# atunnd/Hair-centric-Image-Retrieval

Hardware: AMD Instinct MI355X
Metric: query-images/sec (embed+top-10) ViT-B/16 vs 1M gallery, 1/2/4/8 GPU (higher is better)
Workload: dtype f16; 1 GPU; ViT-B/16 (HSimCLR ViTWrapper, random init) embed + top-10 over 1000000 x 768 f32 gallery row-sharded over 1 GPU(s); query_batch_per_gpu=880, global_query_batch=880, gallery_rows=1000000, gallery_dtype=f32, topk=10, sim_mode=filtered, residual_stream=f16, steps_in_flight=2, parallelism=gallery-shard1+query-dp1

## Files before the change

hair-centric-image-retrieval_amd/csrc/sim_topk.hip:

```cpp
#include "sim_core.h"
#include <math.h>
#include <stdlib.h>

constexpr int kScanAux = 2;

#ifdef HCIR_DIAG_STAMPS
__device__ unsigned long long g_stamps[1024 * 8];
#define HCIR_STAMP(i)                                                                              \
  do {                                                                                             \
    if (!a.floor_val && threadIdx.x == 0 && blockIdx.x < 512)                                      \
      g_stamps[(blockIdx.y * 512 + blockIdx.x) * 8 + (i)] = __builtin_amdgcn_s_memrealtime();     \
  } while (0)
#else
#define HCIR_STAMP(i) \
  do {                \
  } while (0)
#endif

namespace {

constexpr float kNegInf = -__builtin_huge_valf();

template <int KP>
__device__ __forceinline__ void topk_insert(float (&v)[KP], int (&id)[KP], float s, int i) {
// ... 127 lines not shown
    }
    myq[qt] = q_row0 + wave_q * (32 * QT) + qt * 32 + r;
    const bool live = myq[qt] < a.nq;
    const int64_t qc = live ? myq[qt] : q_last;
    qnv[qt] = a.qn ? a.qn[qc] : 1.0f;
    thr[qt] = a.floor_val ? a.floor_val[qc] : kNegInf;
    if constexpr (CAND) {
      for (int gidx = 1; gidx < a.floor_groups; ++gidx) thr[qt] = fminf(thr[qt], a.floor_val[gidx * a.nq + qc]);
      if (!live) thr[qt] = __builtin_huge_valf();
    }
    cval[qt] = a.ceil_val ? a.ceil_val[qc] : __builtin_huge_valf();
    cidx[qt] = a.ceil_val ? a.ceil_idx[qc] : -1;
  }
  float floorv[QT];
#pragma unroll
  for (int qt = 0; qt < QT; ++qt) floorv[qt] = thr[qt];

  const int nkc = (a.d + EPS - 1) / EPS;
  const int64_t nrows = a.row_end - a.row_begin;
  const int64_t ntiles = (nrows + Cfg::GM - 1) / Cfg::GM;
  const int64_t my_tiles = blockIdx.x < ntiles ? (ntiles - blockIdx.x + gridDim.x - 1) / gridDim.x : 0;
  const int64_t nsteps = my_tiles * nkc;
  const int64_t g_last = a.row_end - 1;

  f32x16 acc[2][QT];
#pragma unroll
  for (int gt = 0; gt < 2; ++gt)
#pragma unroll
    for (int qt = 0; qt < QT; ++qt)
#pragma unroll
      for (int i = 0; i < 16; ++i) acc[gt][qt][i] = 0.f;

  u32x4 regs[GLDS ? 1 : Cfg::NLOAD];
  auto tile_row0 = [&](int64_t ti) { return a.row_begin + ((int64_t)blockIdx.x + ti * gridDim.x) * Cfg::GM; };
  constexpr int NPG = Cfg::GM / 32, NPQ = Cfg::QB / 32;
  static_assert(NPG + NPQ == Cfg::NLOAD, "pieces");
  constexpr int EPC_ = SimElem<T>::kPerChunk;
  uint32_t goff[NPG], qoff[NPQ];
  auto set_goff = [&](int64_t rows_valid) {
#pragma unroll
    for (int i = 0; i < NPG; ++i) {
      const int slot = tid + Cfg::NT * i;
      int row = slot >> 3;
      const int chunk = (slot & 7) ^ ((row >> 1) & 7);
      row = row < rows_valid ? row : (int)rows_valid - 1;
      goff[i] = (uint32_t)(((int64_t)row * a.d + chunk * EPC_) * (int64_t)sizeof(T));
    }
  };
  if constexpr (GLDS) {
    set_goff(Cfg::GM);
#pragma unroll
    for (int i = 0; i < NPQ; ++i) {
      const int slot = tid + Cfg::NT * (NPG + i);
      const int row = (slot >> 3) - Cfg::GM;
      const int chunk = (slot & 7) ^ (((slot >> 3) >> 1) & 7);
      int64_t qr = q_row0 + row;
      qr = qr > q_last ? q_last : qr;
      qoff[i] = (uint32_t)(((qr - q_row0) * a.d + chunk * EPC_) * (int64_t)sizeof(T));
    }
  }
  int64_t issue_tile = 0;
  int issue_kc = 0;
  auto issue_stage = [&](int slot) {
    const int64_t r0 = tile_row0(issue_tile);
    if (issue_kc == 0 && r0 + Cfg::GM > a.row_end) set_goff(a.row_end - r0);
    const char* gb = reinterpret_cast<const char*>(g) + (r0 * a.d) * (int64_t)sizeof(T) + issue_kc * 128;
    const char* qb = reinterpret_cast<const char*>(q) + (q_row0 * a.d) * (int64_t)sizeof(T) + issue_kc * 128;
    char* dst = lds + slot * Cfg::STAGE_BYTES + (tid & ~63) * 16;
#pragma unroll
    for (int i = 0; i < NPG; ++i) {
      if (a.shared_stream || kScanAux == 0)
        lds_dma16_v(gb + goff[i], lds_addr(dst) + Cfg::NT * i * 16);
      else
        lds_dma16_v_nt(gb + goff[i], lds_addr(dst) + Cfg::NT * i * 16);
    }
#pragma unroll
    for (int i = 0; i < NPQ; ++i) lds_dma16_v(qb + qoff[i], lds_addr(dst) + Cfg::NT * (NPG + i) * 16);
    if (++issue_kc == nkc) {
      issue_kc = 0;
      ++issue_tile;
    }
  };
  if (nsteps > 0) {
    if constexpr (GLDS) {
#pragma unroll
      for (int s0 = 0; s0 < NST - 1; ++s0)
        if (s0 < nsteps) issue_stage(s0);
    } else {
      sim_stage_load<T, Cfg>(regs, g, tile_row0(0), g_last, q, q_row0, q_last, a.d, 0, tid);
      sim_stage_store<Cfg>(regs, lds, tid);
    }
  }
  if constexpr (!GLDS) __syncthreads();
  HCIR_STAMP(1);

  int64_t tile_i = 0;
  int kc = 0;
  int cur = 0;
  for (int64_t step = 0; step < nsteps; ++step) {
    int nkc_next = kc + 1;
    int64_t ntile_i = tile_i;
    if (nkc_next == nkc) {
      nkc_next = 0;
      ntile_i = tile_i + 1;
    }
    const bool has_next = step + 1 < nsteps;
    if constexpr (GLDS) {
      if (NST > 2 && !a.gn && step + NST - 1 <= nsteps) {
        if constexpr (NST == 4) asm volatile("s_waitcnt vmcnt(%0)" ::"n"(2 * Cfg::NLOAD) : "memory");
        __syncthreads();
      } else {
        sim_glds_retire_and_sync();
      }
      if (step == 0) HCIR_STAMP(2);
      if (step + NST - 1 < nsteps) issue_stage((cur + NST - 1) % NST);
      sim_stage_mfma<T, Cfg, QT>(acc, lds + cur * Cfg::STAGE_BYTES, wave_g, wave_q, lane);
      if (step == nsteps - 1) HCIR_STAMP(3);
    } else {
      if (has_next)
        sim_stage_load<T, Cfg>(regs, g, tile_row0(ntile_i), g_last, q, q_row0, q_last, a.d, nkc_next, tid);
      sim_stage_mfma<T, Cfg, QT>(acc, lds + cur * Cfg::STAGE_BYTES, wave_g, wave_q, lane);
      if (has_next) sim_stage_store<Cfg>(regs, lds + (cur ^ 1) * Cfg::STAGE_BYTES, tid);
    }

    if (kc == nkc - 1) {
      const int64_t row0 = tile_row0(tile_i);
#pragma unroll
      for (int gt = 0; gt < 2; ++gt) {
        const int64_t rbase = row0 + wave_g * 64 + gt * 32 + 4 * h;
        float gnv[16];
        if (a.gn) {
#pragma unroll
          for (int i = 0; i < 16; ++i) {
            const int64_t row = rbase + (i & 3) + 8 * (i >> 2);
            gnv[i] = a.gn[row < a.row_end ? row : g_last];
          }
        }
#pragma unroll
        for (int qt = 0; qt < QT; ++qt) {
          unsigned mask = 0;
#pragma unroll
          for (int i = 0; i < 16; ++i) {
            const int64_t row = rbase + (i & 3) + 8 * (i >> 2);
            float s = acc[gt][qt][i];
            if (a.gn) s = s * gnv[i];
            if (a.qn) s = s * qnv[qt];
            acc[gt][qt][i] = s;
            bool cand = (row < a.row_end) && (s > thr[qt]);
            if constexpr (CAND) cand = cand || ((row < a.row_end) && a.floor_inclusive && s == thr[qt]);
            if (a.ceil_val)
              cand = cand && ((s < cval[qt]) || (s == cval[qt] && (int)row > cidx[qt]));
            mask |= cand ? (1u << i) : 0u;
          }
          unsigned any = 0u;
          if (__ballot(mask != 0u) != 0ull) {
            any = mask;
#pragma unroll
            for (int off = 32; off > 0; off >>= 1) any |= __shfl_xor(any, off);
            any = __builtin_amdgcn_readfirstlane(any);
          }
          if constexpr (!CAND && BATCH) {
            if (__builtin_popcount(any) >= kBatchMin) {
              uint64_t bk[16];
#pragma unroll
              for (int i = 0; i < 16; ++i) {
                const bool c = ((mask >> i) & 1u) && acc[gt][qt][i] > thr[qt];
                bk[i] = c ? merge_key(acc[gt][qt][i], (int)(rbase + (i & 3) + 8 * (i >> 2))) : 0ull;
              }
              key_bitonic_sort16_desc(bk);
              uint64_t lk[KP];
#pragma unroll
              for (int j = 0; j < KP; ++j) lk[j] = merge_key(lv[qt][j], li[qt][j]);
#pragma unroll
              for (int j = 0; j < 16; ++j) {
                const uint64_t o = bk[15 - j];
                lk[KP - 16 + j] = o > lk[KP - 16 + j] ? o : lk[KP - 16 + j];
              }
              key_bitonic_merge_desc<KP>(lk);
#pragma unroll
              for (int j = 0; j < KP; ++j) {
                lv[qt][j] = lk[j] ? merge_key_val(lk[j]) : kNegInf;
                li[qt][j] = lk[j] ? merge_key_idx(lk[j]) : -1;
              }
              thr[qt] = fmaxf(floorv[qt], topk_kth<KP>(lv[qt], a.k));
              any = 0u;
            }
          }
          while (any != 0u) {
            const int i = __builtin_ctz(any);
            any &= any - 1u;
            const float s = acc[gt][qt][i];
            if constexpr (CAND) {
              if ((mask >> i) & 1u) {
                const int pos = atomicAdd(a.cand_cnt + myq[qt], 1);
                if (pos < a.cap) {
                  const int64_t at = a.cand_query_major ? myq[qt] * a.cap + pos : (int64_t)pos * a.nq + myq[qt];
                  a.cand_val[at] = s;
                  a.cand_idx[at] = (int)(rbase + (i & 3) + 8 * (i >> 2));
                } else {
                  *a.overflow = 1;
                }
              }
            } else {
              if (((mask >> i) & 1u) && s > thr[qt]) {
                topk_insert<KP>(lv[qt], li[qt], s, (int)(rbase + (i & 3) + 8 * (i >> 2)));
                thr[qt] = fmaxf(floorv[qt], topk_kth<KP>(lv[qt], a.k));
              }
            }
          }
#pragma unroll
          for (int i = 0; i < 16; ++i) acc[gt][qt][i] = 0.f;
        }
      }
    }
    if constexpr (!GLDS) __syncthreads();
    kc = nkc_next;
    tile_i = ntile_i;
    cur = (cur + 1 == NST) ? 0 : cur + 1;
  }
  HCIR_STAMP(4);
  if constexpr (!CAND) {
  __syncthreads();

  float* mv = reinterpret_cast<float*>(lds);
  int* mi = reinterpret_cast<int*>(lds + QR * NSRC * KP * 4);
  for (int q0r = 0; q0r < Cfg::QB; q0r += QR) {
#pragma unroll
    for (int qt = 0; qt < QT; ++qt) {
      const int ql = wave_q * (32 * QT) + qt * 32 + r - q0r;
      const int src = wave_g * 2 + h;
      if (ql >= 0 && ql < QR) {
#pragma unroll
        for (int j = 0; j < KP; ++j) {
          mv[(ql * NSRC + src) * KP + j] = lv[qt][j];
          mi[(ql * NSRC + src) * KP + j] = li[qt][j];
        }
      }
    }
    __syncthreads();
    if (tid < QR && q_row0 + q0r + tid < a.nq) {
      const float* lv = mv + tid * NSRC * KP;
      const int* li = mi + tid * NSRC * KP;
      uint64_t hk[NSRC];
      int hp[NSRC];
#pragma unroll
      for (int s = 0; s < NSRC; ++s) {
        hp[s] = 0;
        hk[s] = merge_key(lv[s * KP], li[s * KP]);
      }
      float* ov = a.part_val + ((int64_t)blockIdx.x * a.nq + q_row0 + q0r + tid) * KP;
      int* oi = a.part_idx + ((int64_t)blockIdx.x * a.nq + q_row0 + q0r + tid) * KP;
      for (int o0 = 0; o0 < KP; o0 += 16) {
        float ovr[16];
        int oir[16];
#pragma unroll
        for (int o = 0; o < 16; ++o) {
          uint64_t best = hk[0];
          int bs = 0;
#pragma unroll
          for (int s = 1; s < NSRC; ++s) {
            const bool take = hk[s] > best;
            best = take ? hk[s] : best;
            bs = take ? s : bs;
          }
          ovr[o] = best ? merge_key_val(best) : kNegInf;
          oir[o] = best ? merge_key_idx(best) : -1;
          int np = 0;
#pragma unroll
          for (int s = 0; s < NSRC; ++s) np = (s == bs) ? hp[s] + 1 : np;
          const bool more = best != 0ull && np < KP;
          const int at = bs * KP + (more ? np : 0);
          const uint64_t nk = more ? merge_key(lv[at], li[at]) : 0ull;
#pragma unroll
          for (int s = 0; s < NSRC; ++s) {
            const bool upd = best != 0ull && s == bs;
            hp[s] = upd ? np : hp[s];
            hk[s] = upd ? nk : hk[s];
          }
        }
#pragma unroll
        for (int o = 0; o < 16; o += 4) {
          *reinterpret_cast<f32x4*>(ov + o0 + o) = (f32x4){ovr[o], ovr[o + 1], ovr[o + 2], ovr[o + 3]};
          *reinterpret_cast<u32x4*>(oi + o0 + o) =
              (u32x4){(uint32_t)oir[o], (uint32_t)oir[o + 1], (uint32_t)oir[o + 2], (uint32_t)oir[o + 3]};
        }
      }
    }
    __syncthreads();
  }
  }
  HCIR_STAMP(5);
}

struct BigScanArgs {
  const void* q;
  const void* g;
  const float* floor_val;
  float* cand_val;
  int* cand_idx;
  int* cand_cnt;
  int* overflow;
  int64_t nq, row_begin, row_end;
  int d, cap;
};

template <typename T>
__global__ __launch_bounds__(512, 2) void sim_scan_big_kernel(BigScanArgs a) {
  constexpr int STAGE = 512 * 128;
  __shared__ __attribute__((aligned(16))) char lds[2 * STAGE];
  const int tid = threadIdx.x, lane = tid & 63, wave = tid >> 6;
  const int wave_g = wave >> 2, wave_q = wave & 3;
  const int r = lane & 31, h = lane >> 5;
  const int64_t q_row0 = (int64_t)blockIdx.y * 256;
  const int nkc = a.d / 64;
  const int64_t nrows = a.row_end - a.row_begin;
  const int64_t ntiles = (nrows + 255) / 256;
  const int64_t my_tiles =
      (int64_t)blockIdx.x < ntiles ? (ntiles - blockIdx.x + gridDim.x - 1) / gridDim.x : 0;
  const int64_t nsteps = my_tiles * nkc;
  auto tile_row0 = [&](int64_t ti) { return a.row_begin + ((int64_t)blockIdx.x + ti * gridDim.x) * 256; };

  float flo[2];
  int64_t myq[2];
#pragma unroll
  for (int qt = 0; qt < 2; ++qt) {
    myq[qt] = q_row0 + wave_q * 64 + qt * 32 + r;
    flo[qt] = myq[qt] < a.nq ? a.floor_val[myq[qt]] : __builtin_huge_valf();
  }

  const char* qbase = static_cast<const char*>(a.q) + q_row0 * a.d * (int64_t)sizeof(T);
  const char* gbase = nullptr;
  uint32_t goff[4], qoff[4];
#pragma unroll
  for (int i = 0; i < 4; ++i) {
    const int piece = tid + 512 * (4 + i);
    const int row = (piece >> 3) - 256, chunk = (piece & 7) ^ ((((piece >> 3)) >> 1) & 7);
    int64_t qr = row;
    qr = q_row0 + qr > a.nq - 1 ? a.nq - 1 - q_row0 : qr;
    qoff[i] = (uint32_t)((qr * a.d + chunk * 8) * (int64_t)sizeof(T));
  }
  int64_t issue_tile = 0;
  int issue_kc = 0;
  auto set_gallery_sources = [&](int64_t ti) {
    const int64_t r0 = tile_row0(ti);
    gbase = static_cast<const char*>(a.g) + r0 * a.d * (int64_t)sizeof(T);
#pragma unroll
    for (int i = 0; i < 4; ++i) {
      const int piece = tid + 512 * i;
      const int row = piece >> 3, chunk = (piece & 7) ^ ((row >> 1) & 7);
      int64_t gr = row;
      gr = r0 + gr > a.row_end - 1 ? a.row_end - 1 - r0 : gr;
      goff[i] = (uint32_t)((gr * a.d + chunk * 8) * (int64_t)sizeof(T));
    }
  };
  auto issue_piece = [&](int slot, int i) {
    lds_dma16((i < 4 ? gbase : qbase) + issue_kc * 128, i < 4 ? goff[i & 3] : qoff[i & 3],
              lds_addr(lds) + slot * STAGE + ((tid & ~63) + 512 * i) * 16);
  };
  auto issue_advance = [&]() {
    if (++issue_kc == nkc) {
      issue_kc = 0;
      ++issue_tile;
      if (issue_tile < my_tiles) set_gallery_sources(issue_tile);
    }
  };

  f32x16 acc[4][2];
#pragma unroll
  for (int gt = 0; gt < 4; ++gt)
#pragma unroll
    for (int qt = 0; qt < 2; ++qt)
#pragma unroll
      for (int i = 0; i < 16; ++i) acc[gt][qt][i] = 0.f;

  if (nsteps > 0) {
    set_gallery_sources(0);
#pragma unroll
    for (int i = 0; i < 8; ++i) issue_piece(0, i);
    issue_advance();
  }

  int kc = 0;
  int64_t ti = 0;
  for (int64_t step = 0; step < nsteps; ++step) {
    asm volatile("s_waitcnt vmcnt(0)" ::: "memory");
    __builtin_amdgcn_s_barrier();
    const char* st = lds + (step & 1) * STAGE;
    const bool do_issue = step + 1 < nsteps;
    const int islot = (int)((step + 1) & 1);
#pragma unroll
    for (int ks = 0; ks < 4; ++ks) {
      const int chunk = 2 * ks + h;
      u32x4 af[4], bf[2];
#pragma unroll
      for (int gt = 0; gt < 4; ++gt)
        af[gt] = *reinterpret_cast<const u32x4*>(st + sim_slot_off(wave_g * 128 + gt * 32 + r, chunk));
#pragma unroll
      for (int qt = 0; qt < 2; ++qt)
        bf[qt] = *reinterpret_cast<const u32x4*>(st + sim_slot_off(256 + wave_q * 64 + qt * 32 + r, chunk));
      if (do_issue && ks < 2) {
#pragma unroll
        for (int i = 0; i < 4; ++i) issue_piece(islot, 4 * ks + i);
      }
#pragma unroll
      for (int gt = 0; gt < 4; ++gt)
#pragma unroll
        for (int qt = 0; qt < 2; ++qt) {
          if constexpr (__is_same(T, _Float16))
            acc[gt][qt] = __builtin_amdgcn_mfma_f32_32x32x16_f16(__builtin_bit_cast(f16x8, af[gt]),
                                                                 __builtin_bit_cast(f16x8, bf[qt]), acc[gt][qt], 0, 0, 0);
          else
            acc[gt][qt] = __builtin_amdgcn_mfma_f32_32x32x16_bf16(__builtin_bit_cast(bf16x8, af[gt]),
                                                                  __builtin_bit_cast(bf16x8, bf[qt]), acc[gt][qt], 0, 0, 0);
        }
    }
    if (do_issue) issue_advance();

    if (++kc == nkc) {
      const int64_t row0 = tile_row0(ti) + wave_g * 128;
#pragma unroll
      for (int gt = 0; gt < 4; ++gt) {
        const int64_t rbase = row0 + gt * 32 + 4 * h;
#pragma unroll
        for (int qt = 0; qt < 2; ++qt) {
          unsigned mask = 0;
#pragma unroll
          for (int i = 0; i < 16; ++i) {
            const int64_t row = rbase + (i & 3) + 8 * (i >> 2);
            const bool cand = (row < a.row_end) && (acc[gt][qt][i] > flo[qt]);
            mask |= cand ? (1u << i) : 0u;
          }
          if (__ballot(mask != 0u) != 0ull) {
            unsigned any = mask;
#pragma unroll
            for (int off = 32; off > 0; off >>= 1) any |= __shfl_xor(any, off);
            any = __builtin_amdgcn_readfirstlane(any);
            while (any != 0u) {
              const int i = __builtin_ctz(any);
              any &= any - 1u;
              const float sc = acc[gt][qt][i];
              if ((mask >> i) & 1u) {
                const int pos = atomicAdd(a.cand_cnt + myq[qt], 1);
                if (pos < a.cap) {
                  a.cand_val[(int64_t)pos * a.nq + myq[qt]] = sc;
                  a.cand_idx[(int64_t)pos * a.nq + myq[qt]] = (int)(rbase + (i & 3) + 8 * (i >> 2));
                } else {
                  *a.overflow = 1;
                }
              }
            }
          }
#pragma unroll
          for (int i = 0; i < 16; ++i) acc[gt][qt][i] = 0.f;
        }
      }
      kc = 0;
      ++ti;
    }
  }
}

constexpr int kMergeLPL = 9;

template <typename IdxT>
struct MergeArgs {
  const float* vals;
  const IdxT* idx;
  float* out_val;
  int64_t* out_idx;
  int* out_idx32;
  float* kth_val;
  int* kth_idx;
  int64_t nq, idx_base;
  int nlists, kin, kout;
  const float* extra_val;
  const int* extra_idx;
  int kin_extra;
  const int* nlists_q;
  const int* gate;
  int gate_want;
  int* zero_cnt;
  int ngroups;
};

template <typename IdxT, int LPL = kMergeLPL>
__global__ __launch_bounds__(256) void topk_merge_kernel(MergeArgs<IdxT> a) {
  const int lane = threadIdx.x & 63;
  const int64_t qi = (int64_t)blockIdx.x * 4 + (threadIdx.x >> 6);
  if (qi >= a.nq) return;
  if (a.gate && ((*a.gate != 0) != (a.gate_want != 0))) return;
  if (a.zero_cnt && lane == 0) {
    a.zero_cnt[qi] = 0;
    if (qi == 0) a.zero_cnt[a.nq] = 0;
  }
  const bool has_extra = a.extra_val != nullptr;
  int nl = a.nlists;
  if (a.nlists_q) nl = a.nlists_q[qi] < nl ? a.nlists_q[qi] : nl;
  const int total = a.nlists + (has_extra ? 1 : 0);

  float cv[LPL];
  int64_t ci[LPL];
  int hd[LPL];
  auto fetch = [&](int list, int pos, float& v, int64_t& id) {
    v = kNegInf;
    id = -1;
    if (list < a.nlists) {
      if (pos < a.kin && list < nl) {
        const int64_t o = ((int64_t)list * a.nq + qi) * a.kin + pos;
        v = a.vals[o];
        id = (int64_t)a.idx[o];
      }
    } else if (list < total) {
      if (pos < a.kin_extra) {
        v = a.extra_val[qi * a.kin_extra + pos];
        id = a.extra_idx[qi * a.kin_extra + pos];
      }
    }
    if (id < 0) v = kNegInf;
  };
#pragma unroll
  for (int j = 0; j < LPL; ++j) {
    hd[j] = 0;
    fetch(lane + 64 * j, 0, cv[j], ci[j]);
  }
  float keep_v = kNegInf;
  int64_t keep_i = -1;
  for (int o = 0; o < a.kout; ++o) {
    float bv = cv[0];
    int64_t bi = ci[0];
    int bj = 0;
#pragma unroll
    for (int j = 1; j < LPL; ++j) {
      const bool take = (ci[j] >= 0) && (bi < 0 || better(cv[j], ci[j], bv, bi));
      bv = take ? cv[j] : bv;
      bi = take ? ci[j] : bi;
      bj = take ? j : bj;
    }
    float wv = bv;
    int64_t wi = bi;
    int wl = lane;
#pragma unroll
    for (int off = 32; off > 0; off >>= 1) {
      const float ov = __shfl_xor(wv, off);
      const int64_t oi = __shfl_xor(wi, off);
      const int ol = __shfl_xor(wl, off);
      const bool take = (oi >= 0) && (wi < 0 || better(ov, oi, wv, wi));
      wv = take ? ov : wv;
      wi = take ? oi : wi;
      wl = take ? ol : wl;
    }
    if (lane == (o & 63)) {
      keep_v = wv;
      keep_i = wi;
    }
    if ((o & 63) == 63 || o == a.kout - 1) {
      const int oo = (o & ~63) + lane;
      if (oo <= o) {
        a.out_val[qi * a.kout + oo] = keep_i < 0 ? kNegInf : keep_v;
        if (a.out_idx) a.out_idx[qi * a.kout + oo] = keep_i < 0 ? -1 : keep_i + a.idx_base;
        if (a.out_idx32) a.out_idx32[qi * a.kout + oo] = (int)keep_i;
        if (oo == a.kout - 1) {
          if (a.kth_val) a.kth_val[qi] = keep_i < 0 ? kNegInf : keep_v;
          if (a.kth_idx) a.kth_idx[qi] = (int)keep_i;
        }
      }
    }
    if (lane == wl && wi >= 0) {
#pragma unroll
      for (int j = 0; j < LPL; ++j) {
        if (j == bj) {
          hd[j] += 1;
          fetch(lane + 64 * j, hd[j], cv[j], ci[j]);
        }
      }
    }
  }
}

template <int CTRL>
__device__ __forceinline__ uint64_t dpp_max_u64(uint64_t v) {
  const uint32_t lo = (uint32_t)__builtin_amdgcn_update_dpp(0, (int)(uint32_t)v, CTRL, 0xF, 0xF, true);
  const uint32_t hi = (uint32_t)__builtin_amdgcn_update_dpp(0, (int)(uint32_t)(v >> 32), CTRL, 0xF, 0xF, true);
  const uint64_t o = ((uint64_t)hi << 32) | lo;
  return o > v ? o : v;
}
__device__ __forceinline__ uint64_t wave_max_u64(uint64_t v) {
  v = dpp_max_u64<0xB1>(v);
  v = dpp_max_u64<0x4E>(v);
  v = dpp_max_u64<0x141>(v);
  v = dpp_max_u64<0x140>(v);
  uint64_t m = 0;
#pragma unroll
  for (int row = 0; row < 4; ++row) {
    const uint32_t lo = (uint32_t)__builtin_amdgcn_readlane((int)(uint32_t)v, 16 * row);
    const uint32_t hi = (uint32_t)__builtin_amdgcn_readlane((int)(uint32_t)(v >> 32), 16 * row);
    const uint64_t o = ((uint64_t)hi << 32) | lo;
    m = o > m ? o : m;
  }
  return m;
}

template <int LPL>
__global__ __launch_bounds__(256) void topk_merge32_kernel(MergeArgs<int> a) {
  const int lane = threadIdx.x & 63;
  const int64_t qi = (int64_t)blockIdx.x * 4 + (threadIdx.x >> 6);
  if (qi >= a.nq) return;
  if (a.gate && ((*a.gate != 0) != (a.gate_want != 0))) return;
  const int ng_ = a.ngroups > 1 ? a.ngroups : 1, grp = (int)blockIdx.y;
  if (a.zero_cnt && lane == 0 && grp == 0) {
    a.zero_cnt[qi] = 0;
    if (qi == 0) a.zero_cnt[a.nq] = 0;
  }
  const bool has_extra = a.extra_val != nullptr;
  int nl = (a.nlists - grp + ng_ - 1) / ng_;
  if (a.nlists_q) nl = a.nlists_q[qi] < nl ? a.nlists_q[qi] : nl;
  const int extra_list = nl;
  const int64_t gout = (int64_t)grp * a.nq;

  auto fetch4 = [&](int list, int pos, uint64_t (&k4)[4]) {
#pragma unroll
    for (int e = 0; e < 4; ++e) k4[e] = 0ull;
    const float* pv = nullptr;
    const int* pi = nullptr;
    int len = 0;
    if (list < nl) {
      pv = a.vals + ((int64_t)(list * ng_ + grp) * a.nq + qi) * a.kin;
      pi = a.idx + ((int64_t)(list * ng_ + grp) * a.nq + qi) * a.kin;
      len = a.kin;
    } else if (has_extra && list == extra_list) {
      pv = a.extra_val + qi * a.kin_extra;
      pi = a.extra_idx + qi * a.kin_extra;
      len = a.kin_extra;
    }
    if (pos + 4 <= len && (len & 3) == 0) {
      const f32x4 v = *reinterpret_cast<const f32x4*>(pv + pos);
      const u32x4 id = *reinterpret_cast<const u32x4*>(pi + pos);
#pragma unroll
      for (int e = 0; e < 4; ++e) k4[e] = merge_key(v[e], (int)id[e]);
    } else {
#pragma unroll
      for (int e = 0; e < 4; ++e)
        if (pos + e < len) k4[e] = merge_key(pv[pos + e], pi[pos + e]);
    }
  };

  uint64_t kq[LPL][4];
  int used[LPL];
#pragma unroll
  for (int j = 0; j < LPL; ++j) {
    used[j] = 0;
    fetch4(lane + 64 * j, 0, kq[j]);
  }
  uint64_t mine = 0ull;
  for (int o = 0; o < a.kout; ++o) {
    uint64_t best = kq[0][0];
    int bj = 0;
#pragma unroll
    for (int j = 1; j < LPL; ++j) {
      const bool take = kq[j][0] > best;
      best = take ? kq[j][0] : best;
      bj = take ? j : bj;
    }
    const uint64_t wm = wave_max_u64(best);
    mine = (lane == (o & 63)) ? wm : mine;
    if ((o & 63) == 63 || o == a.kout - 1) {
      const int oo = (o & ~63) + lane;
      if (oo <= o) {
        const bool none = mine == 0ull;
        const float wv = none ? kNegInf : merge_key_val(mine);
        const int wi = none ? -1 : merge_key_idx(mine);
        a.out_val[(gout + qi) * a.kout + oo] = wv;
        if (a.out_idx) a.out_idx[(gout + qi) * a.kout + oo] = none ? -1 : (int64_t)wi + a.idx_base;
        if (a.out_idx32) a.out_idx32[(gout + qi) * a.kout + oo] = wi;
        if (oo == a.kout - 1) {
          if (a.kth_val) a.kth_val[gout + qi] = wv;
          if (a.kth_idx) a.kth_idx[gout + qi] = wi;
        }
      }
    }
    if (wm != 0ull && best == wm) {
#pragma unroll
      for (int j = 0; j < LPL; ++j) {
        if (j == bj) {
          kq[j][0] = kq[j][1];
          kq[j][1] = kq[j][2];
          kq[j][2] = kq[j][3];
          kq[j][3] = 0ull;
          used[j] += 1;
          if ((used[j] & 3) == 0) fetch4(lane + 64 * j, used[j], kq[j]);
        }
      }
    }
  }
}

template <int LPL>
__global__ __launch_bounds__(256) void topk_merge32q_kernel(MergeArgs<int> a) {
  __shared__ uint64_t part[4][16];
  const int lane = threadIdx.x & 63, wave = threadIdx.x >> 6;
  const int64_t qi = blockIdx.x;
  if (a.gate && ((*a.gate != 0) != (a.gate_want != 0))) return;
  if (a.zero_cnt && threadIdx.x == 0) {
    a.zero_cnt[qi] = 0;
    if (qi == 0) a.zero_cnt[a.nq] = 0;
  }
  const bool has_extra = a.extra_val != nullptr;
  int nl = a.nlists;
  if (a.nlists_q) nl = a.nlists_q[qi] < nl ? a.nlists_q[qi] : nl;
  const int extra_list = nl;

  auto fetch4 = [&](int list, int pos, uint64_t (&k4)[4]) {
#pragma unroll
    for (int e = 0; e < 4; ++e) k4[e] = 0ull;
    const float* pv = nullptr;
    const int* pi = nullptr;
    int len = 0;
    if (list < nl) {
      pv = a.vals + ((int64_t)list * a.nq + qi) * a.kin;
      pi = a.idx + ((int64_t)list * a.nq + qi) * a.kin;
      len = a.kin;
    } else if (has_extra && list == extra_list) {
      pv = a.extra_val + qi * a.kin_extra;
      pi = a.extra_idx + qi * a.kin_extra;
      len = a.kin_extra;
    }
    if (pos + 4 <= len && (len & 3) == 0) {
      const f32x4 v = *reinterpret_cast<const f32x4*>(pv + pos);
      const u32x4 id = *reinterpret_cast<const u32x4*>(pi + pos);
#pragma unroll
      for (int e = 0; e < 4; ++e) k4[e] = merge_key(v[e], (int)id[e]);
    } else {
#pragma unroll
      for (int e = 0; e < 4; ++e)
        if (pos + e < len) k4[e] = merge_key(pv[pos + e], pi[pos + e]);
    }
  };
  uint64_t kq[LPL][4];
  int used[LPL];
#pragma unroll
  for (int j = 0; j < LPL; ++j) {
    used[j] = 0;
    fetch4(wave + 4 * (lane + 64 * j), 0, kq[j]);
  }
  uint64_t mine = 0ull;
  for (int o = 0; o < a.kout; ++o) {
    uint64_t best = kq[0][0];
    int bj = 0;
#pragma unroll
    for (int j = 1; j < LPL; ++j) {
      const bool take = kq[j][0] > best;
      best = take ? kq[j][0] : best;
      bj = take ? j : bj;
    }
    const uint64_t wm = wave_max_u64(best);
    mine = (lane == o) ? wm : mine;
    if (wm != 0ull && best == wm) {
#pragma unroll
      for (int j = 0; j < LPL; ++j) {
        if (j == bj) {
          kq[j][0] = kq[j][1];
          kq[j][1] = kq[j][2];
// ... 421 lines not shown
  size_t off = 0;
  auto take = [&](size_t n) {
    char* r = c ? c + off : nullptr;
    off += (n + 255) & ~size_t(255);
    return r;
  };
  const size_t part = (size_t)kMaxParts * nq * p.kp;
  w.part_val = reinterpret_cast<float*>(take(part * 4));
  w.part_idx = reinterpret_cast<int*>(take(part * 4));
  w.pre_val = reinterpret_cast<float*>(take((size_t)nq * p.kp * 4));
  w.pre_idx = reinterpret_cast<int*>(take((size_t)nq * p.kp * 4));
  w.floor_val = reinterpret_cast<float*>(take((size_t)nq * 4 * kMaxFloorGroups));
  w.ceil_val = reinterpret_cast<float*>(take((size_t)nq * 4));
  w.ceil_idx = reinterpret_cast<int*>(take((size_t)nq * 4));
  const size_t ccap = (k > 16 && k <= 64 && nq <= 128) ? kCandCapBig : kCandCap;
  w.cand_val = reinterpret_cast<float*>(take(ccap * nq * 4));
  w.cand_idx = reinterpret_cast<int*>(take(ccap * nq * 4));
  w.cand_cnt = reinterpret_cast<int*>(take(((size_t)nq + 1) * 4));
  w.bytes = off;
  return w;
}

template <typename T, int KP, int QT, int WQ, int WGG>
void launch_scan_cfg(const ScanArgs& a, int grid_x, int grid_y, hipStream_t st) {
  if (QT == 1 && a.d % SimElem<T>::kPerStage == 0 && !a.floor_val)
    hipLaunchKernelGGL((sim_topk_scan<T, KP, QT, WQ, WGG, true, false, (QT == 1)>), dim3(grid_x, grid_y), dim3(256), 0,
                       st, a);
  else if (a.d % SimElem<T>::kPerStage == 0)
    hipLaunchKernelGGL((sim_topk_scan<T, KP, QT, WQ, WGG, true>), dim3(grid_x, grid_y), dim3(256), 0, st, a);
  else
    hipLaunchKernelGGL((sim_topk_scan<T, KP, QT, WQ, WGG, false>), dim3(grid_x, grid_y), dim3(256), 0, st, a);
}

template <typename T>
void launch_scan(const Plan& p, const ScanArgs& a, int grid_x, hipStream_t st) {
  const int grid_y = (int)hcir_cdiv(a.nq, p.qb);
  if (p.kp == 64) {
    launch_scan_cfg<T, 64, 1, 1, 4>(a, grid_x, grid_y, st);
  } else if (p.kp == 32) {
    if (p.qb == 32)
      launch_scan_cfg<T, 32, 1, 1, 4>(a, grid_x, grid_y, st);
    else if (p.qb == 64)
      launch_scan_cfg<T, 32, 2, 1, 4>(a, grid_x, grid_y, st);
    else
      launch_scan_cfg<T, 32, 2, 2, 2>(a, grid_x, grid_y, st);
  } else if (p.qb == 32) {
    launch_scan_cfg<T, 16, 1, 1, 4>(a, grid_x, grid_y, st);
  } else if (p.qb == 64) {
    launch_scan_cfg<T, 16, 1, 2, 2>(a, grid_x, grid_y, st);
  } else {
    launch_scan_cfg<T, 16, 2, 2, 2>(a, grid_x, grid_y, st);
  }
}

template <typename T, int QT, int WQ, int WGG>
void launch_cand_cfg(const ScanArgs& a, int grid_x, int grid_y, hipStream_t st) {
  if (a.d % SimElem<T>::kPerStage == 0)
    hipLaunchKernelGGL((sim_topk_scan<T, 16, QT, WQ, WGG, true, true>), dim3(grid_x, grid_y), dim3(256), 0, st, a);
  else
    hipLaunchKernelGGL((sim_topk_scan<T, 16, QT, WQ, WGG, false, true>), dim3(grid_x, grid_y), dim3(256), 0, st, a);
}
template <typename T>
void launch_cand(int qb, const ScanArgs& a, int grid_x, hipStream_t st) {
  const int grid_y = (int)hcir_cdiv(a.nq, qb);
  if (qb == 32)
    launch_cand_cfg<T, 1, 1, 4>(a, grid_x, grid_y, st);
  else if (qb == 64)
    launch_cand_cfg<T, 1, 2, 2>(a, grid_x, grid_y, st);
  else
    launch_cand_cfg<T, 2, 2, 2>(a, grid_x, grid_y, st);
}
void launch_cand_dtype(int dtype, int qb, const ScanArgs& a, int grid_x, hipStream_t st) {
  if (dtype == HCIR_F32)
    launch_cand<float>(qb, a, grid_x, st);
  else if (dtype == HCIR_F16)
    launch_cand<_Float16>(qb, a, grid_x, st);
  else
    launch_cand<__bf16>(qb, a, grid_x, st);
}

void launch_scan_dtype(int dtype, const Plan& p, const ScanArgs& a, int grid_x, hipStream_t st) {
  if (dtype == HCIR_F32)
    launch_scan<float>(p, a, grid_x, st);
  else if (dtype == HCIR_F16)
    launch_scan<_Float16>(p, a, grid_x, st);
  else
    launch_scan<__bf16>(p, a, grid_x, st);
}

}

extern "C" {

#ifdef HCIR_DIAG_STAMPS
int hcir_debug_stamps(unsigned long long* host_dst) {
  return (int)hipMemcpyFromSymbol(host_dst, HIP_SYMBOL(g_stamps), sizeof(unsigned long long) * 1024 * 8);
}
#endif

size_t hcir_sim_topk_workspace_bytes(int64_t nq, int64_t ng, int32_t d, int32_t k, int dtype) {
  (void)d;
  (void)dtype;
  if (nq <= 0 || ng <= 0 || k <= 0) return 0;
  const Plan p = make_plan(nq, ng, k);
  return carve(nullptr, nq, k, p).bytes;
}

int hcir_sim_topk(const void* q, int64_t nq, const void* g, int64_t ng, int32_t d, int32_t k,
                  int dtype, const float* q_inv_norm, const float* g_inv_norm, int64_t idx_base,
                  float* out_val, int64_t* out_idx, void* workspace, size_t workspace_bytes,
                  void* stream) {
  HCIR_ENTER();
  if (!q || !g || !out_val || !out_idx) return HCIR_ERR_INVALID;
  if (nq <= 0 || ng <= 0 || d <= 0 || (d & 7) || k <= 0 || k > HCIR_TOPK_MAX) return HCIR_ERR_INVALID;
  if (k > ng || ng >= (int64_t(1) << 31)) return HCIR_ERR_INVALID;
  if (dtype != HCIR_F32 && dtype != HCIR_F16 && dtype != HCIR_BF16) return HCIR_ERR_UNSUPPORTED;
  const Plan p = make_plan(nq, ng, k);
  Workspace w = carve(workspace, nq, k, p);
  if (!workspace || workspace_bytes < w.bytes) return HCIR_ERR_WORKSPACE;
  hipStream_t st = static_cast<hipStream_t>(stream);
  const int merge_grid = (int)hcir_cdiv(nq, 4);

  const int64_t qblocks = hcir_cdiv(nq, p.qb);
  ScanArgs a{};
  a.q = q;
  a.g = g;
  a.qn = q_inv_norm;
  a.gn = g_inv_norm;
  a.part_val = w.part_val;
  a.part_idx = w.part_idx;
  a.nq = nq;
  a.d = d;
  a.shared_stream = qblocks > 1 ? 1 : 0;

  const int* fallback_gate = nullptr;
  bool prefix_done = false;
  int64_t cand_prefix = 0;
  if (p.npass == 1 && p.prefix < ng && nq <= 128 && (k > 16 || nq <= 32)) {
    const int G = k <= 16 ? 1 : (k + 15) / 16;
    int cap = k <= 16 ? kCandCap : kCandCapBig;
    Plan pc = p;
    pc.kp = 16;
    pc.qb = nq <= 32 ? 32 : (nq <= 64 ? 64 : 128);
    pc.gm = pc.qb == 128 ? 128 : 256;
    int64_t S = p.prefix;
    if (G == 1) {
      S = pc.qb == 32 ? ng / 8 : ng / 16;
      S = S < 8192 ? 8192 : (S > 131072 ? 131072 : S);
      S = hcir_cdiv(S, pc.gm) * pc.gm;
      if (S < ng && 38 * ((ng - S) / S + 1) <= 64 * 7) cap = 64 * 7;
    }
    if (G > 1) {
      const float per = 38.0f * G;
      int64_t rp1 = (int64_t)((float)cap / per);
      rp1 = rp1 < 2 ? 2 : rp1;
      S = hcir_cdiv(ng, rp1);
      S = S < 8192 ? 8192 : S;
      S = hcir_cdiv(S, pc.gm) * pc.gm;
    }
    if (S < ng && hcir_cdiv(S, pc.gm) >= 4 * G) {
      const int64_t qbl = hcir_cdiv(nq, pc.qb);
      ScanArgs c = a;
      c.shared_stream = qbl > 1 ? 1 : 0;
      c.k = G == 1 ? k : 16;
      c.row_begin = 0;
      c.row_end = S;
      const int gm_a = pc.qb == 64 ? 128 : pc.gm;
      const int grid_a = scan_grid_x(hcir_cdiv(S, gm_a), qbl);
      launch_scan_dtype(dtype, pc, c, grid_a, st);
      HCIR_LAUNCH_CHECK();
      MergeArgs<int> m{};
      m.vals = w.part_val;
      m.idx = w.part_idx;
      m.nq = nq;
      m.nlists = grid_a;
      m.kin = 16;
      m.kout = c.k;
      m.out_val = w.pre_val;
      m.out_idx32 = w.pre_idx;
      m.kth_val = w.floor_val;
      m.zero_cnt = w.cand_cnt;
      m.ngroups = G;
      if (G == 1)
        launch_merge32(m, st);
      else
        hipLaunchKernelGGL(topk_merge_sel_kernel<kMergeLPL>, dim3(merge_grid, G), dim3(256), 0, st, m);
      HCIR_LAUNCH_CHECK();
      int* overflow = w.cand_cnt + nq;
      c.row_begin = G == 1 ? S : 0;
      c.row_end = ng;
      c.floor_val = w.floor_val;
      c.floor_groups = G;
      c.floor_inclusive = G > 1 ? 1 : 0;
      c.cand_val = w.cand_val;
      c.cand_idx = w.cand_idx;
      c.cand_cnt = w.cand_cnt;
      c.overflow = overflow;
      c.cap = cap;
      c.cand_query_major = 1;
      const bool cg3 = pc.qb == 64;
      const int grid_b = scan_grid_x(hcir_cdiv(c.row_end - c.row_begin, cg3 ? 128 : pc.gm), qbl, cg3 ? 768 : kMaxGridX);
      launch_cand_dtype(dtype, pc.qb, c, grid_b, st);
      HCIR_LAUNCH_CHECK();
      SelectArgs sa{};
      sa.cand_val = w.cand_val;
      sa.cand_idx = w.cand_idx;
      sa.cand_cnt = w.cand_cnt;
      sa.cap = cap;
      if (G == 1) {
        sa.pre_val = w.pre_val;
        sa.pre_idx = w.pre_idx;
        sa.kpre = k;
      }
      sa.out_val = out_val;
      sa.out_idx = out_idx;
      sa.nq = nq;
      sa.idx_base = idx_base;
      sa.k = k;
      sa.gate = overflow;
      sa.gate_want = 0;
      if (cap == 64 * 7)
        hipLaunchKernelGGL(topk_select_kernel<8>, dim3(merge_grid), dim3(256), 0, st, sa);
      else if (k <= 16)
        hipLaunchKernelGGL(topk_select_kernel<kCandLPL>, dim3(merge_grid), dim3(256), 0, st, sa);
      else
        hipLaunchKernelGGL(topk_select4_kernel<(kCandCapBig + 255) / 256 + 1>, dim3((unsigned)nq), dim3(256), 0, st, sa);
      HCIR_LAUNCH_CHECK();
      fallback_gate = overflow;
      prefix_done = G == 1;
      if (G == 1) cand_prefix = S;
    }
  }

  Plan pp = p;
  if (cand_prefix) pp.prefix = cand_prefix;
  if (fallback_gate && !prefix_done) pp.prefix = ng;
  const bool big = p.npass == 1 && p.prefix < ng && dtype != HCIR_F32 && nq > 128 && k <= 16 &&
                   d % 64 == 0 && !q_inv_norm && !g_inv_norm && ng - p.prefix >= 4096;
  if (big) {
    int64_t rr = (int64_t)((float)kCandCap / ((float)k + 5.0f * sqrtf((float)k)));
    rr = rr > 15 ? 15 : rr;
    int64_t s = hcir_cdiv(ng, (rr < 1 ? 1 : rr) + 1);
    s = s < 8192 ? 8192 : s;
    s = hcir_cdiv(s, p.gm) * p.gm;
    if (s < pp.prefix) pp.prefix = s;
  }
  if (p.npass == 1) {
    a.k = k;
    const bool two_phase = pp.prefix < ng;
    a.row_begin = 0;
    a.row_end = pp.prefix;
    const int64_t tiles_a = hcir_cdiv(pp.prefix, p.gm);
    const int grid_a = scan_grid_x(tiles_a, qblocks);
    a.gate = fallback_gate;
    if (!prefix_done) {
      launch_scan_dtype(dtype, p, a, grid_a, st);
      HCIR_LAUNCH_CHECK();
    }
    MergeArgs<int> m{};
    m.gate = fallback_gate;
    m.gate_want = 1;
    m.vals = w.part_val;
    m.idx = w.part_idx;
    m.nq = nq;
    m.nlists = grid_a;
    m.kin = p.kp;
    m.kout = k;
    if (!two_phase) {
      m.out_val = out_val;
      m.out_idx = out_idx;
      m.idx_base = idx_base;
      launch_merge32(m, st);
      HCIR_LAUNCH_CHECK();
      return HCIR_OK;
    }
    m.out_val = w.pre_val;
    m.out_idx32 = w.pre_idx;
    m.kth_val = w.floor_val;
    if (big) m.zero_cnt = w.cand_cnt;
    if (!prefix_done) {
      launch_merge32(m, st);
      HCIR_LAUNCH_CHECK();
    }
    a.row_begin = pp.prefix;
    a.row_end = ng;
    a.floor_val = w.floor_val;
    int* overflow = w.cand_cnt + nq;
    if (big) {
      BigScanArgs b{};
      b.q = q;
      b.g = g;
      b.floor_val = w.floor_val;
      b.cand_val = w.cand_val;
      b.cand_idx = w.cand_idx;
      b.cand_cnt = w.cand_cnt;
      b.overflow = overflow;
      b.nq = nq;
      b.row_begin = pp.prefix;
      b.row_end = ng;
      b.d = d;
      b.cap = kCandCap;
      const int64_t qb256 = hcir_cdiv(nq, 256);
      const int64_t tiles256 = hcir_cdiv(ng - pp.prefix, 256);
      int64_t gx = 256 / qb256;
      gx = gx < 8 ? 8 : (gx & ~int64_t(7));
      gx = tiles256 < gx ? tiles256 : gx;
      if (dtype == HCIR_F16)
        hipLaunchKernelGGL(sim_scan_big_kernel<_Float16>, dim3((unsigned)gx, (unsigned)qb256), dim3(512), 0, st, b);
      else
        hipLaunchKernelGGL(sim_scan_big_kernel<__bf16>, dim3((unsigned)gx, (unsigned)qb256), dim3(512), 0, st, b);
      HCIR_LAUNCH_CHECK();
      MergeArgs<int> mc{};
      mc.vals = w.cand_val;
      mc.idx = w.cand_idx;
      mc.nq = nq;
      mc.nlists = kCandCap;
      mc.nlists_q = w.cand_cnt;
      mc.kin = 1;
      mc.kout = k;
      mc.extra_val = w.pre_val;
      mc.extra_idx = w.pre_idx;
      mc.kin_extra = k;
      mc.out_val = out_val;
      mc.out_idx = out_idx;
      mc.idx_base = idx_base;
      mc.gate = overflow;
      mc.gate_want = 0;
      launch_merge32(mc, st);
      HCIR_LAUNCH_CHECK();
      a.gate = overflow;
    }
    const int64_t tiles_b = hcir_cdiv(ng - pp.prefix, p.gm);
    const bool q64g3 = p.kp == 16 && p.qb == 64;
    const int grid_b = scan_grid_x(tiles_b, qblocks, q64g3 ? kMaxGridQ64 : kMaxGridX);
    launch_scan_dtype(dtype, p, a, grid_b, st);
    HCIR_LAUNCH_CHECK();
    MergeArgs<int> m2{};
    m2.vals = w.part_val;
    m2.idx = w.part_idx;
    m2.nq = nq;
    m2.nlists = grid_b;
    m2.kin = p.kp;
    m2.kout = k;
    m2.extra_val = w.pre_val;
    m2.extra_idx = w.pre_idx;
    m2.kin_extra = k;
    m2.out_val = out_val;
    m2.out_idx = out_idx;
    m2.idx_base = idx_base;
    if (big) {
      m2.gate = overflow;
      m2.gate_want = 1;
    } else if (fallback_gate) {
      m2.gate = fallback_gate;
      m2.gate_want = 1;
    }
    launch_merge32(m2, st);
    HCIR_LAUNCH_CHECK();
    return HCIR_OK;
  }

  a.row_begin = 0;
  a.row_end = ng;
  const int grid_x = scan_grid_x(hcir_cdiv(ng, p.gm), qblocks);
  int done = 0;
  for (int pass = 0; pass < p.npass; ++pass) {
    const int kk = (k - done) < 64 ? (k - done) : 64;
    a.k = kk;
    a.ceil_val = pass ? w.ceil_val : nullptr;
    a.ceil_idx = pass ? w.ceil_idx : nullptr;
    launch_scan_dtype(dtype, p, a, grid_x, st);
    HCIR_LAUNCH_CHECK();
    MergeArgs<int> m{};
    m.vals = w.part_val;
    m.idx = w.part_idx;
    m.nq = nq;
    m.nlists = grid_x;
    m.kin = p.kp;
    m.kout = kk;
    m.out_val = w.pre_val;
    m.out_idx32 = w.pre_idx;
    m.kth_val = w.ceil_val;
    m.kth_idx = w.ceil_idx;
    hipLaunchKernelGGL(topk_merge32_kernel<kMergeLPL>, dim3(merge_grid), dim3(256), 0, st, m);
    HCIR_LAUNCH_CHECK();
    hipLaunchKernelGGL(pass_copy_kernel, dim3((unsigned)hcir_cdiv(nq * kk, 256)), dim3(256), 0, st,
                       w.pre_val, w.pre_idx, nq, kk, k, done, idx_base, out_val, out_idx);
    HCIR_LAUNCH_CHECK();
    done += kk;
  }
  return HCIR_OK;
}

int hcir_topk_merge(const float* vals, const int64_t* idx, int32_t nlists, int64_t nq, int32_t k_in,
                    int32_t k_out, float* out_val, int64_t* out_idx, void* stream) {
  HCIR_ENTER();
  if (!vals || !idx || !out_val || !out_idx) return HCIR_ERR_INVALID;
  if (nlists <= 0 || nq <= 0 || k_in <= 0 || k_out <= 0) return HCIR_ERR_INVALID;
  if (nlists > 64 * kMergeLPL) return HCIR_ERR_UNSUPPORTED;
  MergeArgs<int64_t> m{};
  m.vals = vals;
  m.idx = idx;
  m.nq = nq;
  m.nlists = nlists;
  m.kin = k_in;
  m.kout = k_out;
  m.out_val = out_val;
  m.out_idx = out_idx;
  m.idx_base = 0;
  hipLaunchKernelGGL(topk_merge_kernel<int64_t>, dim3((int)hcir_cdiv(nq, 4)), dim3(256), 0,
                     static_cast<hipStream_t>(stream), m);
  HCIR_LAUNCH_CHECK();
  return HCIR_OK;
}

int hcir_row_invnorm(const void* x, int64_t n, int32_t d, int64_t ldx, int dtype, float eps,
                     float* out, void* stream) {
  HCIR_ENTER();
  if (!x || !out || n <= 0 || d <= 0 || (d & 3) || ldx < d) return HCIR_ERR_INVALID;
  hipStream_t st = static_cast<hipStream_t>(stream);
  const dim3 grid((unsigned)hcir_cdiv(n, 4)), block(256);
  if (dtype == HCIR_F32)
    hipLaunchKernelGGL(row_invnorm_kernel<float>, grid, block, 0, st, (const float*)x, n, d, ldx, eps, out);
  else if (dtype == HCIR_F16)
    hipLaunchKernelGGL(row_invnorm_kernel<_Float16>, grid, block, 0, st, (const _Float16*)x, n, d, ldx, eps, out);
  else if (dtype == HCIR_BF16)
    hipLaunchKernelGGL(row_invnorm_kernel<__bf16>, grid, block, 0, st, (const __bf16*)x, n, d, ldx, eps, out);
  else
    return HCIR_ERR_UNSUPPORTED;
  HCIR_LAUNCH_CHECK();
  return HCIR_OK;
}

int hcir_l2_normalize(const float* x, int64_t n, int32_t d, float eps, float* y_f32, void* y_f16,
                      void* stream) {
  HCIR_ENTER();
  if (!x || n <= 0 || d <= 0 || (d & 3)) return HCIR_ERR_INVALID;
  hipLaunchKernelGGL(l2_normalize_kernel, dim3((unsigned)hcir_cdiv(n, 4)), dim3(256), 0,
                     static_cast<hipStream_t>(stream), x, n, d, eps, y_f32, (_Float16*)y_f16);
  HCIR_LAUNCH_CHECK();
  return HCIR_OK;
}

int hcir_convert_f32(const float* x, int64_t n, int dtype, void* y, void* stream) {
  HCIR_ENTER();
  if (!x || !y || n <= 0) return HCIR_ERR_INVALID;
  hipStream_t st = static_cast<hipStream_t>(stream);
  int64_t blocks = hcir_cdiv(n, 1024);
  if (blocks > 4096) blocks = 4096;
  if (dtype == HCIR_F16)
    hipLaunchKernelGGL(convert_kernel<_Float16>, dim3((unsigned)blocks), dim3(256), 0, st, x, n, (_Float16*)y);
  else if (dtype == HCIR_BF16)
    hipLaunchKernelGGL(convert_kernel<__bf16>, dim3((unsigned)blocks), dim3(256), 0, st, x, n, (__bf16*)y);
  else
    return HCIR_ERR_UNSUPPORTED;
  HCIR_LAUNCH_CHECK();
  return HCIR_OK;
}

}
```

Baseline: 26030 query-images/sec.

## Specialize tail query block to narrow 128-wide scan with rebalanced grid

When the last 256-query block is at most half full, the scan kernel runs that block with a 128-query-wide body (fewer query loads and accumulators) and splits the fixed 256-block x budget unevenly between full and tail query blocks. The goal is to stop spending a full-width tile's MFMA work and gallery share on a mostly padded tail block. Environment variables select alternate modes, such as separate launches or per-part launches for timing. This adds template variants, extra branching and some env-driven experimental paths.

New measurement: 26020 query-images/sec (median of 3 runs). No clear change (-0.0%).

```diff
diff --git a/hair-centric-image-retrieval_amd/csrc/sim_topk.hip b/hair-centric-image-retrieval_amd/csrc/sim_topk.hip
--- a/hair-centric-image-retrieval_amd/csrc/sim_topk.hip
+++ b/hair-centric-image-retrieval_amd/csrc/sim_topk.hip
@@ -453,23 +453,27 @@
   int* overflow;
   int64_t nq, row_begin, row_end;
   int d, cap;
+  int gx_wide;
+  int gx_narrow;
+  int narrow_y;
+  int y0;
 };
 
-template <typename T>
-__global__ __launch_bounds__(512, 2) void sim_scan_big_kernel(BigScanArgs a) {
+template <typename T, int QW>
+__device__ __forceinline__ void sim_scan_big_body(const BigScanArgs& a, char* lds, const int gx, const int64_t q_row0) {
   constexpr int STAGE = 512 * 128;
-  __shared__ __attribute__((aligned(16))) char lds[2 * STAGE];
+  constexpr int NWQ = QW / 64, GT = NWQ;
+  constexpr int NQP = QW / 64, NP = 4 + NQP;
+  static_assert(QW == 256 || QW == 128, "query width");
   const int tid = threadIdx.x, lane = tid & 63, wave = tid >> 6;
-  const int wave_g = wave >> 2, wave_q = wave & 3;
+  const int wave_g = wave / NWQ, wave_q = wave % NWQ;
   const int r = lane & 31, h = lane >> 5;
-  const int64_t q_row0 = (int64_t)blockIdx.y * 256;
   const int nkc = a.d / 64;
   const int64_t nrows = a.row_end - a.row_begin;
   const int64_t ntiles = (nrows + 255) / 256;
-  const int64_t my_tiles =
-      (int64_t)blockIdx.x < ntiles ? (ntiles - blockIdx.x + gridDim.x - 1) / gridDim.x : 0;
+  const int64_t my_tiles = (int64_t)blockIdx.x < ntiles ? (ntiles - blockIdx.x + gx - 1) / gx : 0;
   const int64_t nsteps = my_tiles * nkc;
-  auto tile_row0 = [&](int64_t ti) { return a.row_begin + ((int64_t)blockIdx.x + ti * gridDim.x) * 256; };
+  auto tile_row0 = [&](int64_t ti) { return a.row_begin + ((int64_t)blockIdx.x + ti * gx) * 256; };
 
   float flo[2];
   int64_t myq[2];
@@ -481,9 +485,9 @@
 
   const char* qbase = static_cast<const char*>(a.q) + q_row0 * a.d * (int64_t)sizeof(T);
   const char* gbase = nullptr;
-  uint32_t goff[4], qoff[4];
-#pragma unroll
-  for (int i = 0; i < 4; ++i) {
+  uint32_t goff[4], qoff[NQP];
+#pragma unroll
+  for (int i = 0; i < NQP; ++i) {
     const int piece = tid + 512 * (4 + i);
     const int row = (piece >> 3) - 256, chunk = (piece & 7) ^ ((((piece >> 3)) >> 1) & 7);
     int64_t qr = row;
@@ -516,9 +520,9 @@
     }
   };
 
-  f32x16 acc[4][2];
-#pragma unroll
-  for (int gt = 0; gt < 4; ++gt)
+  f32x16 acc[GT][2];
+#pragma unroll
+  for (int gt = 0; gt < GT; ++gt)
 #pragma unroll
     for (int qt = 0; qt < 2; ++qt)
 #pragma unroll
@@ -527,7 +531,7 @@
   if (nsteps > 0) {
     set_gallery_sources(0);
 #pragma unroll
-    for (int i = 0; i < 8; ++i) issue_piece(0, i);
+    for (int i = 0; i < NP; ++i) issue_piece(0, i);
     issue_advance();
   }
 
@@ -542,19 +546,19 @@
 #pragma unroll
     for (int ks = 0; ks < 4; ++ks) {
       const int chunk = 2 * ks + h;
-      u32x4 af[4], bf[2];
-#pragma unroll
-      for (int gt = 0; gt < 4; ++gt)
-        af[gt] = *reinterpret_cast<const u32x4*>(st + sim_slot_off(wave_g * 128 + gt * 32 + r, chunk));
+      u32x4 af[GT], bf[2];
+#pragma unroll
+      for (int gt = 0; gt < GT; ++gt)
+        af[gt] = *reinterpret_cast<const u32x4*>(st + sim_slot_off(wave_g * (GT * 32) + gt * 32 + r, chunk));
 #pragma unroll
       for (int qt = 0; qt < 2; ++qt)
         bf[qt] = *reinterpret_cast<const u32x4*>(st + sim_slot_off(256 + wave_q * 64 + qt * 32 + r, chunk));
       if (do_issue && ks < 2) {
 #pragma unroll
-        for (int i = 0; i < 4; ++i) issue_piece(islot, 4 * ks + i);
+        for (int i = 0; i < NP / 2; ++i) issue_piece(islot, NP / 2 * ks + i);
       }
 #pragma unroll
-      for (int gt = 0; gt < 4; ++gt)
+      for (int gt = 0; gt < GT; ++gt)
 #pragma unroll
         for (int qt = 0; qt < 2; ++qt) {
           if constexpr (__is_same(T, _Float16))
@@ -568,9 +572,9 @@
     if (do_issue) issue_advance();
 
     if (++kc == nkc) {
-      const int64_t row0 = tile_row0(ti) + wave_g * 128;
-#pragma unroll
-      for (int gt = 0; gt < 4; ++gt) {
+      const int64_t row0 = tile_row0(ti) + wave_g * (GT * 32);
+#pragma unroll
+      for (int gt = 0; gt < GT; ++gt) {
         const int64_t rbase = row0 + gt * 32 + 4 * h;
 #pragma unroll
         for (int qt = 0; qt < 2; ++qt) {
@@ -608,6 +612,17 @@
       kc = 0;
       ++ti;
     }
+  }
+}
+
+template <typename T>
+__global__ __launch_bounds__(512, 2) void sim_scan_big_kernel(BigScanArgs a) {
+  __shared__ __attribute__((aligned(16))) char lds[2 * 512 * 128];
+  const int y = a.y0 + (int)blockIdx.y;
+  if (y == a.narrow_y) {
+    if ((int)blockIdx.x < a.gx_narrow) sim_scan_big_body<T, 128>(a, lds, a.gx_narrow, (int64_t)y * 256);
+  } else if ((int)blockIdx.x < a.gx_wide) {
+    sim_scan_big_body<T, 256>(a, lds, a.gx_wide, (int64_t)y * 256);
   }
 }
 
@@ -1635,13 +1650,40 @@
       b.cap = kCandCap;
       const int64_t qb256 = hcir_cdiv(nq, 256);
       const int64_t tiles256 = hcir_cdiv(ng - pp.prefix, 256);
-      int64_t gx = 256 / qb256;
+      const bool narrow = qb256 >= 2 && nq - (qb256 - 1) * 256 <= 128;
+      const int mode = getenv("HCIR_TAIL_MODE") ? atoi(getenv("HCIR_TAIL_MODE")) : 1;
+      int64_t gx = 256 / qb256, gxn = 0;
+      if (narrow && mode == 1) gx = (int64_t)(256.0f / ((float)(qb256 - 1) + 0.55f));
+      if (narrow && mode == 2) gx = 256 / (qb256 - 1);
       gx = gx < 8 ? 8 : (gx & ~int64_t(7));
+      if (narrow && mode == 1) gxn = 256 - (qb256 - 1) * gx;
+      if (narrow && mode == 2) gxn = 256;
+      gxn = gxn < 8 && narrow ? 8 : gxn;
+      if (narrow && mode == 1 && getenv("HCIR_TAIL_GXW")) { gx = atoi(getenv("HCIR_TAIL_GXW")); gxn = atoi(getenv("HCIR_TAIL_GXN")); }
+      const int only = getenv("HCIR_TAIL_ONLY") ? atoi(getenv("HCIR_TAIL_ONLY")) : 0;
       gx = tiles256 < gx ? tiles256 : gx;
+      gxn = tiles256 < gxn ? tiles256 : gxn;
+      b.gx_wide = (int)gx;
+      b.gx_narrow = (int)gxn;
+      b.narrow_y = narrow && mode ? (int)qb256 - 1 : -1;
+      auto launch = [&](int64_t x, int64_t y) {
       if (dtype == HCIR_F16)
-        hipLaunchKernelGGL(sim_scan_big_kernel<_Float16>, dim3((unsigned)gx, (unsigned)qb256), dim3(512), 0, st, b);
+        hipLaunchKernelGGL(sim_scan_big_kernel<_Float16>, dim3((unsigned)x, (unsigned)y), dim3(512), 0, st, b);
       else
-        hipLaunchKernelGGL(sim_scan_big_kernel<__bf16>, dim3((unsigned)gx, (unsigned)qb256), dim3(512), 0, st, b);
+        hipLaunchKernelGGL(sim_scan_big_kernel<__bf16>, dim3((unsigned)x, (unsigned)y), dim3(512), 0, st, b);
+      };
+      if (narrow && mode == 2) {
+        launch(gx, qb256 - 1);
+        b.y0 = (int)qb256 - 1;
+        launch(gxn, 1);
+      } else if (only == 1) {
+        launch(gx, qb256 - 1);
+      } else if (only == 2) {
+        b.y0 = (int)qb256 - 1;
+        launch(gxn, 1);
+      } else {
+        launch(gx > gxn ? gx : gxn, qb256);
+      }
       HCIR_LAUNCH_CHECK();
       MergeArgs<int> mc{};
       mc.vals = w.cand_val;
```
